# sag111/ContiniousEnvironment_Follower_Leader

Measured on AMD Instinct MI355X. Metric: env-steps/sec at 65,536 parallel envs; 1/2/4/8 MI355X scaling, higher is better.
Workload: dtype f64

## Files before the change

continiousenvironment_follower_leader_amd/csrc/ftl_frames_group.hpp:

```cpp
#pragma once
#include "ftl_device.hpp"

namespace ftl {

template <int G, int K>
__device__ __forceinline__ int gb_i(int v) {
    if constexpr (G == 4) return __builtin_amdgcn_mov_dpp(v, K * 0x55, 0xf, 0xf, false);
    else if constexpr (G == 8) {
        const int t = __builtin_amdgcn_mov_dpp(v, (K & 3) * 0x55, 0xf, 0xf, false);
        if constexpr (K < 4) return __builtin_amdgcn_update_dpp(t, t, 0x114, 0xf, 0xA, false);
        else return __builtin_amdgcn_update_dpp(t, t, 0x104, 0xf, 0x5, false);
    } else return __shfl(v, (threadIdx.x & ~(G - 1)) + K);
}
template <int G, int K> __device__ __forceinline__ float gb_f(float v) { return __int_as_float(gb_i<G, K>(__float_as_int(v))); }
template <int G, int K> __device__ __forceinline__ double gb_d(double v) {
    return __hiloint2double(gb_i<G, K>(__double2hiint(v)), gb_i<G, K>(__double2loint(v)));
}
__device__ __forceinline__ int gx_i(int v, int off, int G) {
    if (off == 1) return __builtin_amdgcn_mov_dpp(v, 0xB1, 0xf, 0xf, false);
    if (off == 2) return __builtin_amdgcn_mov_dpp(v, 0x4E, 0xf, 0xf, false);
    if (off == 4) {
        const int t = __builtin_amdgcn_update_dpp(v, v, 0x114, 0xf, 0xA, false);
        return __builtin_amdgcn_update_dpp(t, v, 0x104, 0xf, 0x5, false);
    }
    return __shfl_xor(v, off, G);
}
__device__ __forceinline__ float gx_f(float v, int off, int G) { return __int_as_float(gx_i(__float_as_int(v), off, G)); }
__device__ __forceinline__ double gx_d(double v, int off, int G) { return __hiloint2double(gx_i(__double2hiint(v), off, G), gx_i(__double2loint(v), off, G)); }
__device__ __forceinline__ float gx(float v, int off, int G) { return gx_f(v, off, G); }
__device__ __forceinline__ int gx(int v, int off, int G) { return gx_i(v, off, G); }
__device__ __forceinline__ double gx(double v, int off, int G) { return gx_d(v, off, G); }
template <int G> __device__ __forceinline__ double g_up_d(double v, int off) {
    if constexpr (G == 4) {
        const int hi = __double2hiint(v), lo = __double2loint(v);
        if (off == 1) return __hiloint2double(__builtin_amdgcn_mov_dpp(hi, 0x90, 0xf, 0xf, false), __builtin_amdgcn_mov_dpp(lo, 0x90, 0xf, 0xf, false));
        return __hiloint2double(__builtin_amdgcn_mov_dpp(hi, 0x44, 0xf, 0xf, false), __builtin_amdgcn_mov_dpp(lo, 0x44, 0xf, 0xf, false));
    } else if constexpr (G == 8) {
        const int hi = __double2hiint(v), lo = __double2loint(v);
        if (off == 1) return __hiloint2double(__builtin_amdgcn_mov_dpp(hi, 0x111, 0xf, 0xf, false), __builtin_amdgcn_mov_dpp(lo, 0x111, 0xf, 0xf, false));
        if (off == 2) return __hiloint2double(__builtin_amdgcn_mov_dpp(hi, 0x112, 0xf, 0xf, false), __builtin_amdgcn_mov_dpp(lo, 0x112, 0xf, 0xf, false));
        return __hiloint2double(__builtin_amdgcn_mov_dpp(hi, 0x114, 0xf, 0xf, false), __builtin_amdgcn_mov_dpp(lo, 0x114, 0xf, 0xf, false));
    } else return __shfl_up(v, off, G);
}
template <int G> __device__ __forceinline__ float g_pick_f(float v, int k) {
    if constexpr (G == 4) {
        const float a = gb_f<4, 0>(v), b = gb_f<4, 1>(v), c2 = gb_f<4, 2>(v), d = gb_f<4, 3>(v);
        return k == 0 ? a : k == 1 ? b : k == 2 ? c2 : d;
    } else return __shfl(v, k, G);
}
template <int G> __device__ __forceinline__ bool group_any(bool p) {
    unsigned long long m = __ballot(p);
    return ((m >> (threadIdx.x & ~(G - 1))) & ((1ull << G) - 1ull)) != 0ull;
}
template <int G> __device__ __forceinline__ double group_excl_scan(double v, int r, double& total) {
    double incl = v;
#pragma unroll
    for (int off = 1; off < G; off <<= 1) {
        double o = g_up_d<G>(incl, off);
        if (r >= off) incl += o;
    }
    total = gb_d<G, G - 1>(incl);
    return incl - v;
}
template <int G> __device__ __forceinline__ int group_sum(int v) {
#pragma unroll
    for (int off = G / 2; off >= 1; off >>= 1) v += gx(v, off, G);
    return v;
}
template <int G> __device__ __forceinline__ void group_argmin(float& v, int& idx) {
#pragma unroll
    for (int off = G / 2; off >= 1; off >>= 1) {
        float ov = gx(v, off, G);
        int oi = gx(idx, off, G);
        bool take = (ov < v) || (ov == v && oi < idx);
        if (take) { v = ov; idx = oi; }
    }
}

#ifdef FTL_WAVE_TIMES
__device__ unsigned long long g_wt[2 * 8192];
__device__ unsigned int g_wi[8192];
#endif
#ifdef FTL_PROFILE_PATHS
__device__ unsigned long long g_prof[16];
#ifdef FTL_PROFILE_NOCOUNT
#define FTL_PROF(slot, cond, n) do { } while (0)
#else
#define FTL_PROF(slot, cond, n) do { if (cond) atomicAdd(&g_prof[slot], (unsigned long long)(n)); } while (0)
#endif
__device__ unsigned long long g_cyc[16];
__device__ unsigned long long g_cyc_heavy[17];
__device__ unsigned long long g_wave_t[2 * 8192];
__device__ unsigned int g_whist[2][64];
__shared__ unsigned long long s_cyc[16];
#define FTL_TIC(slot) do { unsigned long long _t = __builtin_readcyclecounter(); if (threadIdx.x == 0) s_cyc[slot] += _t - _tprev; _tprev = _t; } while (0)
#define FTL_TIC_INIT unsigned long long _tprev = __builtin_readcyclecounter()
#else
#define FTL_PROF(slot, cond, n) do { } while (0)
#define FTL_TIC(slot) do { } while (0)
#define FTL_TIC_INIT do { } while (0)
#endif

__device__ __forceinline__ unsigned long long d_mix64(unsigned long long x) {
    x ^= x >> 30; x *= 0xBF58476D1CE4E5B9ULL; x ^= x >> 27; x *= 0x94D049BB133111EBULL; x ^= x >> 31; return x;
}
__device__ __forceinline__ double d_uniform01(unsigned long long seed, unsigned long long env_id, unsigned long long resets, unsigned long long frame) {
    unsigned long long key = d_mix64(seed + 0x9E3779B97F4A7C15ULL * (env_id + 1)) ^ d_mix64(0xD1B54A32D192ED03ULL * (resets + 1));
    return (double)(d_mix64(key + 0x9E3779B97F4A7C15ULL * (frame + 1)) >> 11) * (1.0 / 9007199254740992.0);
}

__device__ __forceinline__ int d_stream_id(const FtlDevParams& P, int env) {
    return P.cfg.env_id_base + env + rec_field(P.env_int, P, env)[FTL_EI_STREAM];
}

__device__ __forceinline__ int d_rand_frames(const ftl_config& c, int stream, int resets, int step_count) {
    const double u = d_uniform01(c.rng_seed, (unsigned long long)stream, (unsigned long long)resets,
                                 (unsigned long long)step_count | (1ULL << 40));
    const int v = c.rand_fps_lo + (int)(u * (double)(c.rand_fps_hi - c.rand_fps_lo));
    return v < c.rand_fps_hi ? v : c.rand_fps_hi - 1;
}

struct GCtx {
    int env, r, slot;
    bool valid;
    int scen, cur_target_id, leader_finished, done, crash, is_in_box, is_on_trace, too_close;
    int step_count, finish_timer, traj_len, trk_counter, corr_lo, corr_hi, seed_end, snap_count;
    int error, episodes, green_count, green_len, scan_ok, route_len, near_cnt, snap_head, hint, green_tiny, resets, acc_consumed;
#ifdef FTL_WAVE_TIMES
    int dbg_walk, dbg_full;
#endif
    int err_acc;
    int n_search;
    int fps;
    double acc_penalty, overall_reward, cur_tx, cur_ty;
    double cur_mult, cur_acc, cum_speed;
    float hx, hy;
// ... 141 lines not shown
                    const int k = base + t * FTL_WAVE + lane;
                    const bool v = k < n0L;
                    if (v) dst[k] = q[t];
                    float4 box = v ? make_float4(q[t].x, q[t].y, q[t].x, q[t].y) : make_float4(3.0e38f, 3.0e38f, -3.0e38f, -3.0e38f);
#pragma unroll
                    for (int off = FTL_TRAJ_BLOCK / 2; off >= 1; off >>= 1) {
                        box.x = fminf(box.x, __shfl_xor(box.x, off)); box.y = fminf(box.y, __shfl_xor(box.y, off));
                        box.z = fmaxf(box.z, __shfl_xor(box.z, off)); box.w = fmaxf(box.w, __shfl_xor(box.w, off));
                    }
                    const int k0 = base + t * FTL_WAVE + (lane & ~(FTL_TRAJ_BLOCK - 1));
                    if ((lane & (FTL_TRAJ_BLOCK - 1)) == 0 && k0 < n0L) bbw[k0 / FTL_TRAJ_BLOCK] = box;
                }
            }
        }
    }
    if (go && !wide_copy) {
        float4* bb = reinterpret_cast<float4*>(P.traj_bb) + (size_t)E.env * (c.traj_cap / FTL_TRAJ_BLOCK);
        for (int b = 0; b * FTL_TRAJ_BLOCK < init_n0; b++) {
            float2 q[FTL_TRAJ_BLOCK / G];
#pragma unroll
            for (int t = 0; t < FTL_TRAJ_BLOCK / G; t++) {
                const int k = b * FTL_TRAJ_BLOCK + t * G + E.r;
                q[t] = init_src[k < init_n0 ? k : init_n0 - 1];
            }
            float4 box = make_float4(3.0e38f, 3.0e38f, -3.0e38f, -3.0e38f);
#pragma unroll
            for (int t = 0; t < FTL_TRAJ_BLOCK / G; t++) {
                const int k = b * FTL_TRAJ_BLOCK + t * G + E.r;
                if (k < init_n0) {
                    init_dst[k] = q[t];
                    box.x = fminf(box.x, q[t].x); box.y = fminf(box.y, q[t].y); box.z = fmaxf(box.z, q[t].x); box.w = fmaxf(box.w, q[t].y);
                }
            }
#pragma unroll
            for (int off = G / 2; off >= 1; off >>= 1) {
                box.x = fminf(box.x, gx(box.x, off, G)); box.y = fminf(box.y, gx(box.y, off, G));
                box.z = fmaxf(box.z, gx(box.z, off, G)); box.w = fmaxf(box.w, gx(box.w, off, G));
            }
            if (E.r == 0) bb[b] = box;
        }
    }
    float lpx = gb_f<G, 0>(E.rb.px), lpy = gb_f<G, 0>(E.rb.py);
    if (go) {
        if (E.route_len == 0) { E.done = 1; E.cur_tx = (double)lpx; E.cur_ty = (double)lpy; }
        else { const double2 w = E.route_len > 1 ? rt01[1] : rt01[0]; E.cur_tx = w.x; E.cur_ty = w.y; }
        E.rb.tgt_x = (double)(lpx - 150.0f); E.rb.tgt_y = (double)(lpy - 150.0f); E.rb.dyn_index = 0;
    }
}

template <int G>
__device__ __forceinline__ void g_build_near(const FtlDevParams& P, GCtx& E, int4* s_near, int* s_cnt, float4* s_box) {
    const ftl_config& c = P.cfg;
    const float lpx = gb_f<G, 0>(E.rb.px), lpy = gb_f<G, 0>(E.rb.py), fpx = gb_f<G, 1>(E.rb.px), fpy = gb_f<G, 1>(E.rb.py);
    const float F = (float)(c.rand_fps_hi > 0 ? c.rand_fps_hi : c.frames_per_step);
    const float ml = 0.5f * (float)(c.leader.img_w + c.leader.img_h) + 4.0f + F * (float)fmax(fabs(c.leader.max_speed), fabs(c.leader.min_speed));
    const float mf = 0.5f * (float)(c.follower.img_w + c.follower.img_h) + 4.0f + F * (float)fmax(fabs(c.follower.max_speed), fabs(c.follower.min_speed));
    if (E.r == 0) s_cnt[E.slot] = 0;
    __syncthreads();
    if (E.valid) {
        const int4* src = reinterpret_cast<const int4*>(P.scen.static_rects) + (size_t)E.scen * c.n_static;
        int4* dst = s_near + (size_t)E.slot * c.n_static;
        const float4 box0 = (reinterpret_cast<const float4*>(P.traj_bb) + (size_t)E.env * (c.traj_cap / FTL_TRAJ_BLOCK))[min(E.traj_len, c.traj_cap - 1) / FTL_TRAJ_BLOCK];
        constexpr int SU = 8;
        for (int s0 = 0; s0 < c.n_static; s0 += SU * G) {
            int4 qv[SU];
#pragma unroll
            for (int k = 0; k < SU; k++) { const int s = s0 + k * G + E.r; qv[k] = s < c.n_static ? src[s] : make_int4(0, 0, 0, 0); }
#pragma unroll
            for (int k = 0; k < SU; k++) {
                const int s = s0 + k * G + E.r;
                const int4 q = qv[k];
                float x0 = (float)q.x, x1 = (float)(q.x + q.z), y0 = (float)q.y, y1 = (float)(q.y + q.w);
                bool nl = !(x1 < lpx - ml || x0 > lpx + ml || y1 < lpy - ml || y0 > lpy + ml);
                bool nf = !(x1 < fpx - mf || x0 > fpx + mf || y1 < fpy - mf || y0 > fpy + mf);
                if (s < c.n_static && (nl || nf)) dst[atomicAdd(&s_cnt[E.slot], 1)] = q;
            }
        }
        if (E.r == 0) s_box[E.slot] = box0;
    }
    __syncthreads();
    E.near_cnt = s_cnt[E.slot];
}

__device__ __forceinline__ int g_green_seq(const float2* tr, int n, double maxd) {
    double acc = 0.0; int Gc = 0;
    for (int k = n - 2; k >= 0; k--) {
        float2 cur = tr[k], prev = tr[k + 1];
        acc += euclid_f32(prev.x, prev.y, cur.x, cur.y);
        if (acc <= maxd) Gc++; else break;
    }
    return Gc;
}
static constexpr double kTinySeg = 9.5367431640625e-07;
template <int G>
__device__ __forceinline__ int g_green_walk(const FtlDevParams& P, const GCtx& E, double& wlen, int& tiny) {
    const float2* tr = reinterpret_cast<const float2*>(P.traj + (size_t)E.env * P.cfg.traj_cap * 2);
    const double maxd = P.cfg.max_distance;
    const int n = E.traj_len, cnt = n - 1;
    double base = 0.0, wmax = 0.0; int Gc = 0; bool near = false, small = false;
    for (int it0 = 0; it0 * G < cnt; it0 += 4) {
        float2 cur[4], prev[4];
#pragma unroll
        for (int u = 0; u < 4; u++) {
            int i = (it0 + u) * G + E.r;
            int ic = i < cnt ? i : cnt - 1;
            cur[u] = tr[n - 2 - ic]; prev[u] = tr[n - 1 - ic];
        }
        bool done = false;
#pragma unroll
        for (int u = 0; u < 4; u++) {
            int i = (it0 + u) * G + E.r;
            bool v = i < cnt && !done;
            double d = v ? euclid_f32(prev[u].x, prev[u].y, cur[u].x, cur[u].y) : 0.0;
            double tot;
            double pre = group_excl_scan<G>(d, E.r, tot);
            double val = base + pre + d;
            near |= v && (fabs(val - maxd) < 1e-6);
            small |= v && d != 0.0 && d < kTinySeg;
            Gc += (v && val <= maxd) ? 1 : 0;
            if (v && val <= maxd) wmax = fmax(wmax, val);
            base += tot;
            if (!(base <= maxd)) done = true;
        }
        if (done) break;
    }
    Gc = group_sum<G>(Gc);
#pragma unroll
    for (int off = G / 2; off >= 1; off >>= 1) wmax = fmax(wmax, gx(wmax, off, G));
    tiny = group_any<G>(small) || maxd > 500.0;
    if (tiny && group_any<G>(near)) {
        Gc = g_green_seq(tr, n, maxd);
        wmax = 0.0;
        for (int i = 0; i < Gc; i++) { float2 cur = tr[n - 2 - i], prev = tr[n - 1 - i]; wmax += euclid_f32(prev.x, prev.y, cur.x, cur.y); }
    }
    wlen = wmax;
    return Gc;
}

struct WalkRes { int Gc; double wlen; int tiny; };
__device__ __forceinline__ WalkRes w_green_walk(const float2* tr, int n, double maxd) {
    const int lane = threadIdx.x & (FTL_WAVE - 1), cnt = n - 1;
    double base = 0.0, wmax = 0.0; int Gc = 0; bool near = false, small = false;
    for (int i0 = 0; i0 < cnt; i0 += FTL_WAVE) {
        const int i = i0 + lane, ic = i < cnt ? i : cnt - 1;
        const float2 cur = tr[n - 2 - ic], prev = tr[n - 1 - ic];
        const bool v = i < cnt;
        const double d = v ? euclid_f32(prev.x, prev.y, cur.x, cur.y) : 0.0;
        double incl = d;
#pragma unroll
        for (int off = 1; off < FTL_WAVE; off <<= 1) {
            const double o = __hiloint2double(__shfl_up(__double2hiint(incl), off), __shfl_up(__double2loint(incl), off));
            if (lane >= off) incl += o;
        }
        const double val = base + incl;
        near |= v && (fabs(val - maxd) < 1e-6);
        small |= v && d != 0.0 && d < kTinySeg;
        const unsigned long long in = __ballot(v && val <= maxd);
        const int k = __popcll(in);
        if (k > 0) wmax = __hiloint2double(__builtin_amdgcn_readlane(__double2hiint(val), k - 1), __builtin_amdgcn_readlane(__double2loint(val), k - 1));
        Gc += k;
        base += __hiloint2double(__builtin_amdgcn_readlane(__double2hiint(incl), FTL_WAVE - 1), __builtin_amdgcn_readlane(__double2loint(incl), FTL_WAVE - 1));
        if (!(base <= maxd)) break;
    }
    WalkRes r;
    r.tiny = (__ballot(small) != 0ull) || maxd > 500.0;
    if (r.tiny && __ballot(near) != 0ull) {
// ... 36 lines not shown
    const int b_lo = lo / FTL_TRAJ_BLOCK, b_hi = (hi - 1) / FTL_TRAJ_BLOCK;
    for (int b00 = b_lo; b00 <= b_hi; b00 += FTL_BOX_UNROLL * G) {
        float4 bx[FTL_BOX_UNROLL];
#pragma unroll
        for (int u = 0; u < FTL_BOX_UNROLL; u++) bx[u] = bb[min(b00 + u * G + r, b_hi)];
        float bd2u[FTL_BOX_UNROLL];
#pragma unroll
        for (int u = 0; u < FTL_BOX_UNROLL; u++) {
            const float dx = fmaxf(fmaxf(bx[u].x - px, px - bx[u].z), 0.0f), dy = fmaxf(fmaxf(bx[u].y - py, py - bx[u].w), 0.0f);
            bd2u[u] = (b00 + u * G + r <= b_hi) ? dx * dx + dy * dy - 1e-2f : __int_as_float(0x7f800000);
        }
#pragma unroll
        for (int u = 0; u < FTL_BOX_UNROLL; u++) {
        const int b0 = b00 + u * G;
        const float bd2 = bd2u[u];
        if (b0 > b_hi) break;
        unsigned m = (unsigned)((__ballot(bd2 <= bound) >> (threadIdx.x & ~(G - 1))) & ((1ull << G) - 1ull));
        if (!(bd2 <= bound)) skipmin = fminf(skipmin, bd2);
        while (m) {
            int k = __ffs(m) - 1; m &= m - 1;
            float kd2 = g_pick_f<G>(bd2, k);
            if (!(kd2 <= bound)) { skipmin = fminf(skipmin, kd2); continue; }
            int s0 = (b0 + k) * FTL_TRAJ_BLOCK;
            int i0 = max(s0, lo), i1 = min(s0 + FTL_TRAJ_BLOCK, hi);
            float2 qq[FTL_TRAJ_BLOCK / G];
#pragma unroll
            for (int t = 0; t < FTL_TRAJ_BLOCK / G; t++) qq[t] = tr[min(i0 + r + t * G, i1 - 1)];
#pragma unroll
            for (int t = 0; t < FTL_TRAJ_BLOCK / G; t++) {
                const int i = i0 + r + t * G;
                if (i < i1) {
                    float ddx = qq[t].x - px, ddy = qq[t].y - py;
                    float d2 = ddx * ddx + ddy * ddy;
                    int ky = reversed ? (hi - 1 - i) : i;
                    if (d2 < best || (d2 == best && ky < key)) { best = d2; bi = i; key = ky; bp = qq[t]; }
                }
            }
            float gbest = best;
#pragma unroll
            for (int off = G / 2; off >= 1; off >>= 1) gbest = fminf(gbest, gx(gbest, off, G));
            bound = fminf(bound, gbest);
        }
        }
    }
#pragma unroll
    for (int off = G / 2; off >= 1; off >>= 1) {
        float ov = gx(best, off, G); int ok = gx(key, off, G); int oi = gx(bi, off, G);
        float ox = gx(bp.x, off, G), oy = gx(bp.y, off, G);
        bool take = (ov < best) || (ov == best && ok < key);
        if (take) { best = ov; key = ok; bi = oi; bp.x = ox; bp.y = oy; }
        skipmin = fminf(skipmin, gx(skipmin, off, G));
    }
}

__device__ __forceinline__ int g_cache_class(const ftl_config& c, const GCtx& E, float fpx, float fpy, int fps, bool want_quiet, bool& quiet) {
    const int n = E.traj_len, g_lo = n - 1 - E.green_count;
    const double eps = c.leader_pos_epsilon, mdev = c.max_dev, far = fmax(mdev, eps);
    const float eps2_lo = (float)(eps * eps * (1.0 - 1e-5)), dev2_lo = (float)(mdev * mdev * (1.0 - 1e-5));
    const float eps_hi = (float)(eps * (1.0 + 1e-5)) + 1e-3f, far_hi = (float)(far * (1.0 + 1e-5)) + 1e-3f;
    const bool h_green = E.hint >= g_lo && E.hint <= n - 2;
    const float dx = E.hx - fpx, dy = E.hy - fpy, hd2 = dx * dx + dy * dy;
    int fast = 0;
    if (h_green && hd2 < eps2_lo) fast = 1;
    else if (h_green && hd2 < dev2_lo && E.clr_g > eps_hi) fast = 2;
    else if (E.clr_g > far_hi) fast = (E.clr_a > eps_hi) ? 3 : (hd2 < eps2_lo ? 4 : 0);
    quiet = false;
    if (!want_quiet) return fast;
    const float reach = (float)fps * (float)fmax(fabs(c.follower.max_speed), fabs(c.follower.min_speed)) * 1.001f + 1e-3f;
    const float hd = sqrtf(hd2);
    const bool h_stays_green = E.hint >= g_lo + 2 + fps / c.trajectory_saving_period;
    const float eps_lo = (float)(eps * (1.0 - 1e-5)), dev_lo = (float)(mdev * (1.0 - 1e-5));
    if (fast == 1) quiet = h_stays_green && hd + reach < eps_lo;
    else if (fast == 2) quiet = h_stays_green && hd + reach < dev_lo && E.clr_g - reach > eps_hi;
    else if (fast != 0) quiet = E.clr_g - reach > far_hi && (E.clr_a - reach > eps_hi || hd + reach < eps_lo);
    else quiet = false;
    return fast;
}

enum { FR_TOO_CLOSE = 1, FR_IN_BOX = 2, FR_ON_TRACE = 4, FR_COLLISION = 8, FR_LEADER_HIT = 16, FR_LEADER_FINISHED = 32, FR_TOO_FAR = 64,
       FR_PENDING = 128 };
struct FrPend { float fpx, fpy; unsigned short n, gc, hint, key; };

template <int G, bool REG>
__device__ __forceinline__ void g_frame(const FtlDevParams& P, GCtx& E, const Limits& L, double2& lead_cs, const int4* s_near, int& tick, const bool first, const int f_idx,
                                        unsigned char* s_rec, const int rec_stride, FrPend* s_pend, int* s_pcnt, bool& pend, int& pend_idx, float& new_ad) {
    const ftl_config& c = P.cfg;
    const int r = E.r;
    const bool act = E.valid && r < P.R;
    FTL_TIC_INIT;

    const float lpx0 = gb_f<G, 0>(E.rb.px), lpy0 = gb_f<G, 0>(E.rb.py);
    const float fpx0 = gb_f<G, 1>(E.rb.px), fpy0 = gb_f<G, 1>(E.rb.py);
    const double ldir0 = gb_d<G, 0>(E.rb.direction);
    const int orx = E.rb.rx, ory = E.rb.ry, orw = E.rb.rw, orh = E.rb.rh;

    if (euclid_f64_lt((double)lpx0, (double)lpy0, E.cur_tx, E.cur_ty, c.leader_pos_epsilon)) {
        E.cur_target_id += 1;
        if (E.cur_target_id >= E.route_len) E.leader_finished = 1;
        else {
            const double* rt = P.scen.route + ((size_t)E.scen * c.route_cap + E.cur_target_id) * 2;
            E.cur_tx = rt[0]; E.cur_ty = rt[1];
        }
    }
    FTL_TIC(13);
    double tx = E.cur_tx, ty = E.cur_ty;
    const bool is_bear = act && r >= 2;
#ifndef FTL_BEAR_SINCOS
    const double lc = gb_d<G, 0>(lead_cs.x), ls = gb_d<G, 0>(lead_cs.y);
#endif
    if (is_bear) {
        const int b = r - 2;
        bool near = euclid_f64_lt((double)E.rb.px, (double)E.rb.py, E.rb.tgt_x, E.rb.tgt_y, c.leader_pos_epsilon);
        double off, lvl;
        bool drawn = false;
        if (c.move_bear_v4 && (b & 1)) {
            if (near) E.rb.dyn_index += 1;
            if (E.rb.dyn_index > 3) E.rb.dyn_index = 0;
            drawn = b >= 4;
            const int order = (b == 1) ? 0x2134  : 0x4213 ;
            int p = (order >> (4 * E.rb.dyn_index)) & 0xf;
            lvl = (p <= 2) ? 150.0 : 250.0;
            off = (p == 1) ? 140.0 : (p == 2) ? -140.0 : (p == 3) ? -160.0 : 160.0;
        } else {
            if (near) { E.rb.dyn_index += 1; if (E.rb.dyn_index > 1) E.rb.dyn_index = 0; }
            lvl = 100.0 * (b + 1);
            off = (E.rb.dyn_index == 0) ? -130.0 : 130.0;
        }
        double s, co;
#ifdef FTL_BEAR_SINCOS
        sincos_bounded((ldir0 + off) * kDeg2Rad, s, co);
#else
        {
            const double a = fabs(off);
            const double ca = a == 130.0 ? -0.6427876096865394 : a == 140.0 ? -0.7660444431189779 : -0.9396926207859083;
            const double sa0 = a == 130.0 ? 0.766044443118978 : a == 140.0 ? 0.6427876096865395 : 0.3420201433256689;
            const double sa = off < 0.0 ? -sa0 : sa0;
            co = lc * ca - ls * sa; s = ls * ca + lc * sa;
        }
#endif
        tx = (double)lpx0 + co * lvl; ty = (double)lpy0 + s * lvl;
        if (FTL_MAX_BEARS > 4 && drawn) {
            const int lo = (int)c.max_distance, k = 2 * E.rb.dyn_index;
            auto draw = [&](int kk, int stop) {
                const int nn = (stop - lo + 9) / 10;
                const double u = d_uniform01(c.rng_seed, (unsigned long long)d_stream_id(P, E.env), (unsigned long long)E.resets,
                                             (unsigned long long)E.step_count | (1ULL << 41) | ((unsigned long long)b << 44) | ((unsigned long long)kk << 48));
                const int v = (int)(u * (double)nn);
                return (double)(lo + 10 * (v < nn ? v : nn - 1));
            };
            tx = draw(k, c.width - lo); ty = draw(k + 1, c.height - lo);
        }
        E.rb.tgt_x = tx; E.rb.tgt_y = ty;
    }
    double lspeed = c.leader.max_speed + 0;
    if (REG && !E.leader_finished && (c.n_speed_regime >= 0 || c.n_acc_regime >= 0)) {
        double speed = c.leader.max_speed, acceleration = 0;
        if (c.n_speed_regime >= 0) {
            int sel = -1;
            for (int i = 0; i < c.n_speed_regime; i++) if (c.speed_key[i] <= E.step_count) sel = i;
            if (sel >= 0) {
                if (c.speed_is_range[sel]) {
                    double u = d_uniform01(c.rng_seed, (unsigned long long)d_stream_id(P, E.env), (unsigned long long)E.resets, (unsigned long long)E.step_count);
                    E.cur_mult = c.speed_lo[sel] + (c.speed_hi[sel] - c.speed_lo[sel]) * u;
                } else E.cur_mult = c.speed_lo[sel];
            }
            speed = c.leader.max_speed * E.cur_mult;
        }
        if (c.n_acc_regime >= 0) {
            for (int i = 0; i < c.n_acc_regime; i++)
                if (!((E.acc_consumed >> i) & 1) && c.acc_key[i] <= E.step_count) { E.cur_acc = c.acc_val[i]; E.cum_speed = E.cur_acc; E.acc_consumed |= 1 << i; }
            E.cum_speed += E.cur_acc;
            acceleration = (E.cum_speed * c.leader.max_speed) / E.fps;
        }
        lspeed = speed + acceleration;
    }
    bool steers = (act && r == 0 && !E.leader_finished) || is_bear;
    if (steers) steer_to_point(E.rb, L, tx, ty, r == 0, lspeed);
    if (E.leader_finished) {
        if (r == 0) { command_forward(E.rb, L, 0); command_turn(E.rb, L, 0, 0); }
    }
    bool moves = act && !(r == 0 && E.leader_finished);
    FTL_TIC(14);
    robot_move(E.rb, L, moves, lead_cs.y, lead_cs.x);
    FTL_TIC(15);

    const float fpx = gb_f<G, 1>(E.rb.px), fpy = gb_f<G, 1>(E.rb.py);
    const int frx = gb_i<G, 1>(E.rb.rx), fry = gb_i<G, 1>(E.rb.ry), frw = gb_i<G, 1>(E.rb.rw), frh = gb_i<G, 1>(E.rb.rh);
    const float lpx = gb_f<G, 0>(E.rb.px), lpy = gb_f<G, 0>(E.rb.py);
    const int lrx = gb_i<G, 0>(E.rb.rx), lry = gb_i<G, 0>(E.rb.ry), lrw = gb_i<G, 0>(E.rb.rw), lrh = gb_i<G, 0>(E.rb.rh);
    bool fhit = false, lhit = false;
    for (int s = r; s < E.near_cnt; s += G) {
        int4 q = s_near[s];
        fhit |= rects_collide(frx, fry, frw, frh, q.x, q.y, q.z, q.w);
        lhit |= rects_collide(lrx, lry, lrw, lrh, q.x, q.y, q.z, q.w);
    }
    if (act && r != 1) fhit |= rects_collide(frx, fry, frw, frh, orx, ory, orw, orh);
    if (act && r == 1) lhit |= rects_collide(lrx, lry, lrw, lrh, E.rb.rx, E.rb.ry, E.rb.rw, E.rb.rh);
    fhit = group_any<G>(fhit); lhit = group_any<G>(lhit);
    bool f_coll = false;
    if (!c.ignore_follower_collisions) {
        bool out = (double)fpx > (double)c.width || (double)fpy > (double)c.height || fpx < 0.0f || fpy < 0.0f;
        f_coll = fhit || out;
    }
    FTL_TIC(0);
    const float2* tr = reinterpret_cast<const float2*>(P.traj + (size_t)E.env * c.traj_cap * 2);
#ifndef FTL_ABLATE_GREEN
    bool g_upd = false, g_walk = false; int Gn = 0; double W = 0.0; int tiny = 0;
    if (E.green_len != E.traj_len) {
        g_upd = true;
        const int nn = E.traj_len;
        const double maxd = c.max_distance;
        bool exact = (E.green_len != nn - 1) || (nn % 1024 == 0) || E.green_count < 1;
        Gn = E.green_count + 1; W = E.green_w; tiny = E.green_tiny;
        const double band = tiny ? 1e-6 : 0.0;
        if (!exact) {
            const int o = nn - 2 - Gn;
            float2 p1 = tr[nn - 1], p0 = tr[nn - 2];
            float2 q0 = tr[max(o, 0)], q1 = tr[max(o + 1, 0)], q2 = tr[max(o + 2, 0)], q3 = tr[max(o + 3, 0)];
            asm volatile("" :: "v"(q2.x), "v"(q2.y), "v"(q3.x), "v"(q3.y));
            const double d_beyond = euclid_f32(q1.x, q1.y, q0.x, q0.y), d_old1 = euclid_f32(q2.x, q2.y, q1.x, q1.y),
                         d_old2 = euclid_f32(q3.x, q3.y, q2.x, q2.y);
            const double d_new = euclid_f32(p1.x, p1.y, p0.x, p0.y);
            if (d_new != 0.0 && d_new < kTinySeg) { tiny = 1; exact = true; }
            W += d_new;
            double nxt = d_beyond;
            bool have_nxt = o >= 0;
            if (W > maxd) {
                if (fabs(W - maxd) < band || Gn < 2) exact = true;
                W -= d_old1; Gn -= 1; nxt = d_old1; have_nxt = true;
                if (W > maxd) {
                    if (fabs(W - maxd) < band || Gn < 2) exact = true;
                    W -= d_old2; Gn -= 1; nxt = d_old2;
                    if (W > maxd) exact = true;
                }
            }
            if (fabs(W - maxd) < band) exact = true;
            if (have_nxt && !(W + nxt > maxd + band)) exact = true;
        }
#ifdef FTL_DEBUG_EXACT
        if (exact) { int why = (E.green_len != nn - 1) ? 1 : (E.green_count < 1 ? 2 : 3); E.error = (E.error & 0xff) | (why << 8) | ((((E.error >> 16) + 1) & 0xffff) << 16); }
#endif
#ifdef FTL_WAVE_TIMES
        if (exact) E.dbg_walk += 1;
#endif
        g_walk = exact;
    }
#ifndef FTL_ABLATE_EXACT
    if (REG && c.rand_fps_hi > 0) {
        if (g_walk) Gn = g_green_walk<G>(P, E, W, tiny);
    } else {
        unsigned long long need = __ballot(g_walk && E.valid && r == 0);
        while (need) {
            const int L = __ffsll((long long)need) - 1; need &= need - 1;
            const int envL = __builtin_amdgcn_readlane(E.env, L), nL = __builtin_amdgcn_readlane(E.traj_len, L);
            const WalkRes wr = w_green_walk(reinterpret_cast<const float2*>(P.traj + (size_t)envL * c.traj_cap * 2), nL, c.max_distance);
            if (((int)threadIdx.x & ~(G - 1)) == (L & ~(G - 1))) { Gn = wr.Gc; W = wr.wlen; tiny = wr.tiny; }
        }
    }
#endif
    if (g_upd) { E.green_count = Gn; E.green_w = W; E.green_len = E.traj_len; E.green_tiny = tiny; }
#endif
    FTL_TIC(1);
    const int Gc = E.green_count, n = E.traj_len;
    int rec = f_coll ? FR_COLLISION : 0;
    FTL_PROF(0, E.valid && r == 0, 1);
    {
        float mx = fpx - fpx0, my = fpy - fpy0;
        float disp = sqrtf(mx * mx + my * my) * 1.000001f + 1e-5f;
        E.clr_g -= disp; E.clr_a -= disp;
    }
    pend = false;
    if (Gc > 2) {
        FTL_PROF(1, E.valid && r == 0, 1);
        bool quiet;
        int fast = g_cache_class(c, E, fpx, fpy, E.fps, first, quiet);
        if (first && !quiet) fast = 0;
        FTL_PROF(2, E.valid && r == 0 && fast != 0, 1);
        FTL_PROF(13, E.valid && r == 0 && first && fast == 0, 1);
        FTL_PROF(14, E.valid && r == 0 && !first && fast == 0, 1);
        if (fast == 1) rec |= FR_ON_TRACE | FR_IN_BOX;
        else if (fast == 2) rec |= FR_IN_BOX;
// ... 529 lines not shown
        const size_t e = (size_t)(base + __ffsll((long long)m) - 1); m &= m - 1;
        if (lane < FTL_OBS_NUM) fin.obs_num[e * FTL_OBS_NUM + lane] = out.obs_num[e * FTL_OBS_NUM + lane];
        if (lane < 2) fin.target[2 * e + lane] = out.target[2 * e + lane];
        for (int i = lane; i < lasers_len; i += FTL_WAVE) fin.lasers[e * lasers_len + i] = out.lasers[e * lasers_len + i];
        if (fin.policy_obs)
            for (int i = lane; i < pol_len; i += FTL_WAVE) fin.policy_obs[e * pol_len + i] = out.policy_obs[e * pol_len + i];
    }
}

}

#ifndef FTL_FRAMESG_WPE
#define FTL_FRAMESG_WPE 2
#endif

template <int G, bool REG, bool XR = false>
__global__ void __launch_bounds__(FTL_WAVE, FTL_FRAMESG_WPE) ftl_frames_group_kernel(const FtlDevParams* __restrict__ Pp, const FtlCall C) {
    extern __shared__ __align__(16) unsigned char lds[];
    using namespace ftl;
    const FtlDevParams& P = *Pp;
    constexpr int EPW = FTL_WAVE / G;
    GCtx E;
    E.slot = threadIdx.x / G; E.r = threadIdx.x % G;
    const int gslot = ((int)blockIdx.x * C.parts + C.part) * EPW + E.slot;
    E.valid = gslot < P.n_envs;
    E.env = E.valid ? (P.perm ? P.perm[gslot] : gslot) : P.n_envs - 1;
    int4* s_near = reinterpret_cast<int4*>(lds);
    int* s_cnt = reinterpret_cast<int*>(lds + (size_t)EPW * P.cfg.n_static * 16);
    E.scan_ok = 0; E.near_cnt = 0; E.n_search = 0; E.err_acc = 0;
    const Limits L = lane_limits(P.cfg, E.r);
#ifdef FTL_WAVE_TIMES
    if (threadIdx.x == 0 && blockIdx.x < 8192) g_wt[2 * blockIdx.x] = __builtin_amdgcn_s_memrealtime();
    bool wt_reset = false; E.dbg_walk = 0; E.dbg_full = 0;
#endif
#ifdef FTL_PROFILE_PATHS
    if (threadIdx.x < 16) s_cyc[threadIdx.x] = 0;
    if (threadIdx.x == 0 && blockIdx.x < 8192) g_wave_t[2 * blockIdx.x] = __builtin_amdgcn_s_memrealtime();
    __syncthreads();
#endif
    FTL_TIC_INIT;
    if (C.mode == 1) {
        if (C.mask && !C.mask[E.env]) E.valid = false;
        const bool fin = XR && (C.flags & FTL_CALL_FINISH);
        if (fin && __ballot(E.valid) == 0ull) return;
        g_load<G>(P, E);
        if (E.valid) E.err_acc |= E.error;
        if (fin && E.valid) E.episodes += 1;
        g_reset<G>(P, E, E.valid ? ((fin && !(C.flags & FTL_CALL_SCEN_IDX)) ? C.win_base + ((E.scen % C.win_count) + C.win_stride) % C.win_count : C.scen_idx[E.env]) : E.scen, E.valid);
        if (E.valid && E.r == 0 && !fin) {
            C.out.reward[E.env] = 0.0; C.out.done[E.env] = (uint8_t)E.done;
            C.out.status[3 * (size_t)E.env] = 0; C.out.status[3 * (size_t)E.env + 1] = 0; C.out.status[3 * (size_t)E.env + 2] = 0;
        }
        __syncthreads();
    } else {
#ifdef FTL_NO_LATE_LOAD
        g_load<G>(P, E);
#else
        g_load<G, true, REG>(P, E);
#endif
        bool rs = false;
        if (XR && (C.flags & FTL_STEP_NEXT_RESET)) {
            rs = E.valid && rec_field(P.env_int, P, E.env)[FTL_EI_DONE] != 0;
            if (rs) E.valid = false;
        }
        FTL_TIC(4);
        double a0, a1;
        if (C.action_kind == FTL_ACTION_BOX2) { a0 = C.action[2 * (size_t)E.env]; a1 = C.action[2 * (size_t)E.env + 1]; }
        else if (C.action_kind == FTL_ACTION_DISCRETE) {
            const int k = reinterpret_cast<const int32_t*>(C.action)[E.env];
            const double mr = P.cfg.follower.max_rotation_speed;
            a0 = P.cfg.follower.max_speed;
            a1 = k == 0 ? -mr : k == 1 ? -mr / 2 : k == 3 ? mr / 2 : k == 4 ? mr : 0.0;
            if (k < 0 || k > 4) E.error |= FTL_ERR_BAD_ACTION;
        } else { a0 = 0.25; a1 = C.action[E.env]; }

        g_build_near<G>(P, E, s_near, s_cnt, reinterpret_cast<float4*>(lds + P.fr_env_off + EPW * 4 + 16));
        if (E.r == 1) {
            command_forward(E.rb, L, a0);
            if (a1 < 0) command_turn(E.rb, L, fabs(a1), -1);
            else if (a1 > 0) command_turn(E.rb, L, a1, 1);
            else command_turn(E.rb, L, 0, 0);
        }
        double reward = 0; int i0 = 0, i1 = 0, i2 = 0;
        const int4* near = s_near + (size_t)E.slot * P.cfg.n_static;
        unsigned char* s_rec = lds + P.fr_rec_off;
        const int rec_stride = P.fr_rec_stride;
        FrPend* s_pend = reinterpret_cast<FrPend*>(lds + P.fr_pend_off);
        int* s_env = reinterpret_cast<int*>(lds + P.fr_env_off);
        int* s_pcnt = s_env + EPW;
        if (E.r == 0) s_env[E.slot] = E.env;
        if (threadIdx.x == 0) *s_pcnt = 0;
        const bool defer = P.fr_defer != 0;
        int sc = E.step_count;
        double2 lead_cs;
        sincos_bounded(E.rb.direction * kDeg2Rad, lead_cs.y, lead_cs.x);
        __syncthreads();
        FTL_TIC(5);
        int tick = (E.step_count + 1) % P.cfg.trajectory_saving_period;
#ifdef FTL_ABLATE_FRAMES
        const int f_max = FTL_ABLATE_FRAMES;
#else
        const int f_max = (REG && P.cfg.rand_fps_hi > 0) ? P.cfg.rand_fps_hi - 1 : P.cfg.frames_per_step;
#endif
#pragma nounroll
        for (int f = 0; f < f_max; f++) {
            bool pend = false; int pend_idx = -1; float new_ad = 3.0e38f;
            if (!REG || f < E.fps) g_frame<G, REG>(P, E, L, lead_cs, near, tick, f == 0, f, s_rec, rec_stride, s_pend, s_pcnt, pend, pend_idx, new_ad);
            __syncthreads();
            if (f == 0 || !defer || f == f_max - 1) {
                const int cnt = *s_pcnt;
                if (cnt > 0) {
                    const bool spread = defer && f > 0;
                    int hint; float hx, hy, cg, ca;
                    const int own = pend ? gb_i<G, 0>(pend_idx) : -1;
                    g_resolve<G>(P, E, s_pend, s_rec, rec_stride, s_env, cnt, spread, own, hint, hx, hy, cg, ca);
                    if (pend && !spread) {
                        E.hint = hint;
                        if (hx < 1.0e38f) { E.hx = hx; E.hy = hy; }
                        if (cg >= 0.0f) E.clr_g = fminf(cg, new_ad);
                        if (ca >= 0.0f) E.clr_a = fminf(ca, new_ad);
                    }
                    __syncthreads();
                    if (threadIdx.x == 0) *s_pcnt = 0;
                    __syncthreads();
                }
            }
        }
        FTL_TIC(11);
#ifndef FTL_NO_LATE_LOAD
        g_load_late<REG>(P, E);
#endif
        const int done0 = E.done;
        const TailK TK = tail_consts(P.cfg);
#pragma nounroll
        for (int f0 = 0; f0 < f_max; f0 += 4) {
            const unsigned w = *reinterpret_cast<const unsigned*>(s_rec + E.slot * rec_stride + f0);
#pragma unroll
            for (int j = 0; j < 4; j++) {
                const int f = f0 + j;
                if (f < f_max && (!REG || f < E.fps)) g_tail(TK, E, (int)((w >> (8 * j)) & 255u), sc, reward, i0, i1, i2);
            }
        }
        if (REG && P.cfg.rand_fps_hi > 0) E.fps = d_rand_frames(P.cfg, d_stream_id(P, E.env), E.resets, E.step_count);
        if (E.valid && E.r == 0) {
            C.out.reward[E.env] = reward; C.out.done[E.env] = (uint8_t)E.done;
            C.out.status[3 * (size_t)E.env] = (uint8_t)i0; C.out.status[3 * (size_t)E.env + 1] = (uint8_t)i1; C.out.status[3 * (size_t)E.env + 2] = (uint8_t)i2;
        }
        FTL_TIC(9);
        if (E.valid && E.r == 0 && E.done && (!done0 || (C.flags & (XR ? FTL_STEP_AUTO_RESET | FTL_CALL_DEFER_RESET : FTL_STEP_AUTO_RESET)))) {
            double* st = P.ep_stats + (size_t)E.env * FTL_N_METRICS;
            st[FTL_M_EPISODES] += 1.0; st[FTL_M_RETURN_SUM] += E.overall_reward; st[FTL_M_FRAMES_SUM] += (double)E.step_count;
            if (i0 == FTL_MISSION_SUCCESS) st[FTL_M_SUCCESS] += 1.0;
            if (i1 == FTL_AGENT_CRASH) st[FTL_M_CRASH] += 1.0;
            if (i1 == FTL_AGENT_LOW_REWARD) st[FTL_M_LOW_REWARD] += 1.0;
            if (i1 == FTL_AGENT_TOO_FAR) st[FTL_M_TOO_FAR] += 1.0;
            if (i0 == FTL_MISSION_FINISHED_BY_TIME) st[FTL_M_TIMEOUT] += 1.0;
        }
        bool go = E.valid && E.done && (C.flags & FTL_STEP_AUTO_RESET);
        if (XR) {
            const bool defer = (C.flags & FTL_CALL_DEFER_RESET) != 0;
            if (rs) {
                const int* ei = rec_field(P.env_int, P, E.env);
                E.valid = true;
                E.error = ei[FTL_EI_ERROR]; E.acc_consumed = ei[FTL_EI_ACC_CONSUMED];
                E.fps = P.cfg.rand_fps_hi > 0 ? ei[FTL_EI_FPS] : P.cfg.frames_per_step;
            }
            const bool ended = E.valid && !rs && E.done && (!done0 || defer);
            if (E.valid && E.r == 0) {
                if (C.ended) C.ended[E.env] = ended ? 1 : 0;
                if (C.restarted) C.restarted[E.env] = (rs || (defer && ended)) ? 1 : 0;
            }
            go = rs || (go && !defer);
        }
        if (__ballot(go) != 0ull) {
#ifdef FTL_PROFILE_PATHS
            if (threadIdx.x == 0) s_cyc[12] = 1;
#endif
#ifdef FTL_WAVE_TIMES
            wt_reset = true;
#endif
            if (go) { E.episodes += 1; E.err_acc |= E.error; }
            g_reset<G>(P, E, go ? C.win_base + ((E.scen % C.win_count) + C.win_stride) % C.win_count : E.scen, go);
            if (XR && rs && E.r == 0) {
                C.out.reward[E.env] = 0.0; C.out.done[E.env] = (uint8_t)E.done;
                C.out.status[3 * (size_t)E.env] = 0; C.out.status[3 * (size_t)E.env + 1] = 0; C.out.status[3 * (size_t)E.env + 2] = 0;
            }
            __syncthreads();
        }
    }
    FTL_TIC(6);
// ... 59 lines not shown
```

Baseline: 286.7 million.

## Cache first near-obstacle rect per lane in packed registers; fuse hit reductions

Before the frame loop, each group lane loads its first near-static rectangle and packs it into two 16-bit-pair registers, provided every rect in the wave fits in 16 bits. Each frame then tests collisions against the register copy and walks LDS only when more than G near obstacles exist, or when packing failed. The two separate group_any ballots for follower and leader hits are merged into one group_or over a 2-bit mask, which uses DPP for G=4/8. This removes the repeated per-frame LDS reads and one reduction, at the cost of extra registers and a uniform fallback branch.

```diff
diff --git a/continiousenvironment_follower_leader_amd/csrc/ftl_frames_group.hpp b/continiousenvironment_follower_leader_amd/csrc/ftl_frames_group.hpp
--- a/continiousenvironment_follower_leader_amd/csrc/ftl_frames_group.hpp
+++ b/continiousenvironment_follower_leader_amd/csrc/ftl_frames_group.hpp
@@ -48,10 +48,22 @@
         return k == 0 ? a : k == 1 ? b : k == 2 ? c2 : d;
     } else return __shfl(v, k, G);
 }
-template <int G> __device__ __forceinline__ bool group_any(bool p) {
-    unsigned long long m = __ballot(p);
-    return ((m >> (threadIdx.x & ~(G - 1))) & ((1ull << G) - 1ull)) != 0ull;
-}
+template <int G, int NB> __device__ __forceinline__ int group_or(int v) {
+    if constexpr (G == 4 || G == 8) {
+#pragma unroll
+        for (int off = 1; off < G; off <<= 1) v |= gx_i(v, off, G);
+        return v;
+    } else {
+        int o = 0;
+#pragma unroll
+        for (int b = 0; b < NB; b++) {
+            const unsigned long long m = __ballot(((v >> b) & 1) != 0);
+            if (((m >> (threadIdx.x & ~(G - 1))) & ((1ull << G) - 1ull)) != 0ull) o |= 1 << b;
+        }
+        return o;
+    }
+}
+template <int G> __device__ __forceinline__ bool group_any(bool p) { return group_or<G, 1>(p ? 1 : 0) != 0; }
 template <int G> __device__ __forceinline__ double group_excl_scan(double v, int r, double& total) {
     double incl = v;
 #pragma unroll
@@ -359,6 +371,19 @@
     E.near_cnt = s_cnt[E.slot];
 }
 
+struct NearReg { int xy, wh; };
+template <int G>
+__device__ __forceinline__ NearReg near_regs(const GCtx& E, const int4* near, int& walk_from) {
+    const int4 q = E.r < E.near_cnt ? near[E.r] : make_int4(0, 0, 0, 0);
+    const bool fits = q.x >= -32768 && q.x < 32768 && q.y >= -32768 && q.y < 32768 && (unsigned)q.z < 65536u && (unsigned)q.w < 65536u;
+    const bool packed = __ballot(!fits) == 0ull;
+    walk_from = !packed ? 0 : (__ballot(E.near_cnt > G) != 0ull ? G : -1);
+    NearReg n;
+    n.xy = packed ? (q.x & 0xffff) | (int)((unsigned)q.y << 16) : 0;
+    n.wh = packed ? q.z | (int)((unsigned)q.w << 16) : 0;
+    return n;
+}
+
 __device__ __forceinline__ int g_green_seq(const float2* tr, int n, double maxd) {
     double acc = 0.0; int Gc = 0;
     for (int k = n - 2; k >= 0; k--) {
@@ -561,7 +586,8 @@
 struct FrPend { float fpx, fpy; unsigned short n, gc, hint, key; };
 
 template <int G, bool REG>
-__device__ __forceinline__ void g_frame(const FtlDevParams& P, GCtx& E, const Limits& L, double2& lead_cs, const int4* s_near, int& tick, const bool first, const int f_idx,
+__device__ __forceinline__ void g_frame(const FtlDevParams& P, GCtx& E, const Limits& L, double2& lead_cs, const int4* s_near, const NearReg nq, const int walk_from,
+                                        int& tick, const bool first, const int f_idx,
                                         unsigned char* s_rec, const int rec_stride, FrPend* s_pend, int* s_pcnt, bool& pend, int& pend_idx, float& new_ad) {
     const ftl_config& c = P.cfg;
     const int r = E.r;
@@ -667,15 +693,26 @@
     const int frx = gb_i<G, 1>(E.rb.rx), fry = gb_i<G, 1>(E.rb.ry), frw = gb_i<G, 1>(E.rb.rw), frh = gb_i<G, 1>(E.rb.rh);
     const float lpx = gb_f<G, 0>(E.rb.px), lpy = gb_f<G, 0>(E.rb.py);
     const int lrx = gb_i<G, 0>(E.rb.rx), lry = gb_i<G, 0>(E.rb.ry), lrw = gb_i<G, 0>(E.rb.rw), lrh = gb_i<G, 0>(E.rb.rh);
-    bool fhit = false, lhit = false;
-    for (int s = r; s < E.near_cnt; s += G) {
-        int4 q = s_near[s];
-        fhit |= rects_collide(frx, fry, frw, frh, q.x, q.y, q.z, q.w);
-        lhit |= rects_collide(lrx, lry, lrw, lrh, q.x, q.y, q.z, q.w);
+    const int qx = (nq.xy << 16) >> 16, qy = nq.xy >> 16, qw = nq.wh & 0xffff, qh = (int)((unsigned)nq.wh >> 16);
+    bool fhit = rects_collide(frx, fry, frw, frh, qx, qy, qw, qh);
+    bool lhit = rects_collide(lrx, lry, lrw, lrh, qx, qy, qw, qh);
+    if (walk_from >= 0) {
+        int slot = E.slot;
+        asm volatile("" : "+v"(slot));
+        const int4* nl = s_near + (size_t)slot * c.n_static;
+        const int cnt = reinterpret_cast<const int*>(s_near + (size_t)(FTL_WAVE / G) * c.n_static)[slot];
+        for (int s = r + walk_from; s < cnt; s += G) {
+            int4 q = nl[s];
+            fhit |= rects_collide(frx, fry, frw, frh, q.x, q.y, q.z, q.w);
+            lhit |= rects_collide(lrx, lry, lrw, lrh, q.x, q.y, q.z, q.w);
+        }
     }
     if (act && r != 1) fhit |= rects_collide(frx, fry, frw, frh, orx, ory, orw, orh);
     if (act && r == 1) lhit |= rects_collide(lrx, lry, lrw, lrh, E.rb.rx, E.rb.ry, E.rb.rw, E.rb.rh);
-    fhit = group_any<G>(fhit); lhit = group_any<G>(lhit);
+    {
+        const int hb = group_or<G, 2>((fhit ? 1 : 0) | (lhit ? 2 : 0));
+        fhit = (hb & 1) != 0; lhit = (hb & 2) != 0;
+    }
     bool f_coll = false;
     if (!c.ignore_follower_collisions) {
         bool out = (double)fpx > (double)c.width || (double)fpy > (double)c.height || fpx < 0.0f || fpy < 0.0f;
@@ -1371,7 +1408,8 @@
             else command_turn(E.rb, L, 0, 0);
         }
         double reward = 0; int i0 = 0, i1 = 0, i2 = 0;
-        const int4* near = s_near + (size_t)E.slot * P.cfg.n_static;
+        int walk_from;
+        const NearReg nq = near_regs<G>(E, s_near + (size_t)E.slot * P.cfg.n_static, walk_from);
         unsigned char* s_rec = lds + P.fr_rec_off;
         const int rec_stride = P.fr_rec_stride;
         FrPend* s_pend = reinterpret_cast<FrPend*>(lds + P.fr_pend_off);
@@ -1394,7 +1432,7 @@
 #pragma nounroll
         for (int f = 0; f < f_max; f++) {
             bool pend = false; int pend_idx = -1; float new_ad = 3.0e38f;
-            if (!REG || f < E.fps) g_frame<G, REG>(P, E, L, lead_cs, near, tick, f == 0, f, s_rec, rec_stride, s_pend, s_pcnt, pend, pend_idx, new_ad);
+            if (!REG || f < E.fps) g_frame<G, REG>(P, E, L, lead_cs, s_near, nq, walk_from, tick, f == 0, f, s_rec, rec_stride, s_pend, s_pcnt, pend, pend_idx, new_ad);
             __syncthreads();
             if (f == 0 || !defer || f == f_max - 1) {
                 const int cnt = *s_pcnt;
```

Result: no change. 289.0 million, median of 6 (+0.8%).
